# bcgsc/abyss

Measured on NVIDIA H100. Metric: k-mers/sec (Bloom insert + unitig extend), higher is better.
Workload: dtype u8

## Files before the change

abyss_b200/capi.py:

```python
from __future__ import annotations

import ctypes as C
import os

import numpy as np

_HERE = os.path.dirname(os.path.abspath(__file__))
LIB_PATH = os.path.join(_HERE, "lib", "libabyssb200.so")

ABB_OK, ABB_EINVAL, ABB_ENODEV, ABB_ECUDA, ABB_ENOMEM, ABB_ESTATE = 0, -1, -2, -3, -4, -5
COUNTING, BIT, CASCADING, KONNECTOR = 0, 1, 2, 3


class AbbError(RuntimeError):
    def __init__(self, code: int, msg: str):
        super().__init__(f"libabyssb200 error {code}: {msg}")
        self.code = code


class InsertStats(C.Structure):
    _fields_ = [("kmers", C.c_uint64), ("slots", C.c_uint64), ("windows", C.c_uint64),
                ("deferred", C.c_uint64), ("launches", C.c_uint64),
                ("ms_hash", C.c_float), ("ms_insert", C.c_float), ("ms_commit", C.c_float),
                ("commit_launches", C.c_uint64), ("commit_slots", C.c_uint64), ("drains", C.c_uint64),
                ("drained_slots", C.c_uint64), ("graph_launches", C.c_uint64), ("ms_graph", C.c_float)]


class Contig(C.Structure):
    _fields_ = [("seed_read", C.c_uint64), ("seq_offset", C.c_uint64),
                ("length", C.c_uint32), ("coverage", C.c_uint32)]


class AssemblyParams(C.Structure):
    _fields_ = [("trim", C.c_uint), ("verbose", C.c_uint), ("read_log", C.c_uint), ("reserved", C.c_uint)]


class TraceRow(C.Structure):
    _fields_ = [("contig_id", C.c_uint64), ("seed_read", C.c_uint64), ("length", C.c_uint32), ("seed_pos", C.c_uint32),
                ("left_n", C.c_uint32), ("right_n", C.c_uint32), ("left_code", C.c_uint8), ("right_code", C.c_uint8),
                ("redundant", C.c_uint8), ("pad", C.c_uint8)]


class AssemblyStats(C.Structure):
    _fields_ = [("rounds", C.c_uint64), ("speculated_reads", C.c_uint64), ("wasted_reads", C.c_uint64),
                ("candidates", C.c_uint64), ("contigs_tried", C.c_uint64), ("launches", C.c_uint64),
                ("ms_classify", C.c_float), ("ms_visited", C.c_float), ("ms_extend", C.c_float), ("ms_replay", C.c_float),
                ("ms_tiles", C.c_float), ("ms_walk", C.c_float), ("ms_stage", C.c_float), ("ms_repeat", C.c_float), ("ms_total", C.c_float), ("ms_cand", C.c_float), ("markers", C.c_uint64), ("tiles", C.c_uint64), ("serial_fallbacks", C.c_uint64),
                ("untiled_markers", C.c_uint64), ("dropped_tiles", C.c_uint64)]


class AssemblyCounters(C.Structure):
    _fields_ = [("solid_reads", C.c_uint64), ("visited_reads", C.c_uint64),
                ("reads_processed", C.c_uint64), ("bases_assembled", C.c_uint64),
                ("contig_id", C.c_uint64)]


class SuccInfo(C.Structure):
    _fields_ = [("hash", C.c_uint64 * 4), ("mask", C.c_uint8), ("pad", C.c_uint8 * 7)]


class NbrInfo(C.Structure):
    _fields_ = [("self", C.c_uint64), ("hash", C.c_uint64 * 8), ("attr", C.c_uint32), ("mask", C.c_uint8), ("pad", C.c_uint8 * 3)]


class OverlapEdge(C.Structure):
    _fields_ = [("u", C.c_uint32), ("v", C.c_uint32), ("distance", C.c_int32)]


class OverlapStats(C.Structure):
    _fields_ = [("vertices", C.c_uint64), ("exact_edges", C.c_uint64), ("short_edges", C.c_uint64), ("blunt_vertices", C.c_uint64),
                ("launches", C.c_uint64)]


_u64p = C.POINTER(C.c_uint64)
_u8p = C.POINTER(C.c_uint8)
_vp = C.c_void_p

SIGNATURES = {
    "abb_version": (C.c_int, []),
    "abb_last_error": (C.c_char_p, []),
    "abb_device_count": (C.c_int, []),
    "abb_filter_create": (C.c_int, [C.POINTER(_vp), C.c_int, C.c_uint64, C.c_uint, C.c_uint, C.c_uint, C.c_char_p, C.c_int]),
    "abb_filter_destroy": (C.c_int, [_vp]),
    "abb_konnector_create": (C.c_int, [C.POINTER(_vp), C.c_uint64, C.c_uint, C.c_uint, C.c_uint64, C.c_uint64, C.c_uint64, C.c_int]),
    "abb_filter_read_bits": (C.c_int, [_vp, C.c_int, _vp, C.c_uint64, C.c_uint64, C.c_int]),
    "abb_filter_compare": (C.c_int, [_vp, _vp, _u64p]),
    "abb_filter_level_popcount": (C.c_int, [_vp, C.c_int, _u64p]),
    "abb_filter_kmer_size": (C.c_uint, [_vp]),
    "abb_filter_hash_num": (C.c_uint, [_vp]),
    "abb_filter_size": (C.c_uint64, [_vp]),
    "abb_filter_size_in_bytes": (C.c_uint64, [_vp]),
    "abb_filter_threshold": (C.c_uint, [_vp]),
    "abb_filter_levels": (C.c_uint, [_vp]),
    "abb_filter_set_threshold": (C.c_int, [_vp, C.c_uint]),
    "abb_insert_reads": (C.c_int, [_vp, _vp, _vp, C.c_uint64, _u64p]),
    "abb_insert_reads_dev": (C.c_int, [_vp, _vp, _vp, C.c_uint64, C.c_uint64, _u64p]),
    "abb_insert_hashes": (C.c_int, [_vp, _vp, C.c_uint64]),
    "abb_contains_hashes": (C.c_int, [_vp, _vp, C.c_uint64, _vp]),
    "abb_mincount_hashes": (C.c_int, [_vp, _vp, C.c_uint64, _vp]),
    "abb_hash_reads": (C.c_int, [C.c_uint, C.c_char_p, _vp, _vp, C.c_uint64, _vp, _vp, _u64p, C.c_int]),
    "abb_hash_reads_dev": (C.c_int, [_vp, _vp, _vp, C.c_uint64, _vp, _vp, C.c_uint64, _u64p]),
    "abb_comm_unique_id": (C.c_int, [_vp]),
    "abb_comm_create": (C.c_int, [C.POINTER(_vp), C.c_int, C.c_int, _vp, C.c_int]),
    "abb_comm_destroy": (C.c_int, [_vp]),
    "abb_comm_rank": (C.c_int, [_vp]),
    "abb_comm_world": (C.c_int, [_vp]),
    "abb_insert_reads_sharded_dev": (C.c_int, [_vp, _vp, _vp, _vp, C.c_uint64, C.c_int, _u64p]),
    "abb_insert_reads_sharded": (C.c_int, [_vp, _vp, _vp, _vp, C.c_uint64, C.c_int, _u64p]),
    "abb_filter_resident_reads": (C.c_int, [_vp, C.POINTER(_vp), C.POINTER(_vp), _u64p]),
    "abb_filter_allgather": (C.c_int, [_vp, _vp]),
    "abb_comm_allgather_bytes": (C.c_int, [_vp, _vp, C.c_uint64, _vp]),
    "abb_comm_exchange_bytes": (C.c_int, [_vp, _vp, C.c_uint64, _vp, _u64p, _u64p, _vp]),
    "abb_filter_device_ptr": (_vp, [_vp, C.c_int]),
    "abb_filter_download": (C.c_int, [_vp, C.c_int, _vp, C.c_uint64]),
    "abb_filter_upload": (C.c_int, [_vp, C.c_int, _vp, C.c_uint64]),
    "abb_filter_clear": (C.c_int, [_vp]),
    "abb_filter_popcount": (C.c_int, [_vp, _u64p, _u64p]),
    "abb_assembler_create": (C.c_int, [C.POINTER(_vp), _vp, C.POINTER(AssemblyParams)]),
    "abb_assembler_destroy": (C.c_int, [_vp]),
    "abb_assembler_process_reads": (C.c_int, [_vp, _vp, _vp, C.c_uint64, C.POINTER(C.POINTER(Contig)), _u64p, C.POINTER(C.c_char_p)]),
    "abb_assembler_process_reads_dev": (C.c_int, [_vp, _vp, _vp, C.c_uint64, C.POINTER(C.POINTER(Contig)), _u64p, C.POINTER(C.c_char_p)]),
    "abb_assembler_stats": (C.c_int, [_vp, C.POINTER(AssemblyStats)]),
    "abb_assembler_reset": (C.c_int, [_vp]),
    "abb_assembler_counters": (C.c_int, [_vp, C.POINTER(AssemblyCounters)]),
    "abb_assembler_set_counters": (C.c_int, [_vp, C.POINTER(AssemblyCounters)]),
    "abb_assembler_read_results": (C.c_int, [_vp, C.POINTER(_u8p), _u64p]),
    "abb_assembler_set_comm": (C.c_int, [_vp, _vp]),
    "abb_assembler_trace": (C.c_int, [_vp, C.POINTER(C.POINTER(TraceRow)), _u64p]),
    "abb_assembler_assembled_filter": (_vp, [_vp]),
    "abb_filter_insert_stats": (C.c_int, [_vp, C.POINTER(InsertStats), C.c_int]),
# ... 441 lines not shown
```

abyss_b200/csrc/abb_assemble.cu:

```cuda
#include "abb_common.h"
#include "abb_walk.cuh"
#include <cooperative_groups.h>
#include <cub/device/device_select.cuh>
#include <thrust/iterator/counting_iterator.h>
#include <algorithm>
#include <chrono>
#include <cstdlib>
#include <cstring>
#include <new>
#include <vector>

namespace abb {
namespace cg = cooperative_groups;

__host__ __device__ inline uint64_t tile_slot(uint64_t key, unsigned cls, unsigned mask)
{
	return (((key ^ (0x9E3779B97F4A7C15ULL * (cls + 1))) * 0xD6E8FEB86659FD93ULL) >> 24) & mask;
}

struct WarpCtx {
	unsigned k, trim;
	RollTab rt;
	const HashCfg* cfg;
	const uint8_t* counters;
// ... 317 lines not shown
	unsigned ordinal;
	unsigned len;
	unsigned seed_pos;
	unsigned psize;
	unsigned char left, right, flags, pad1;
	unsigned long long front_h, back_h;
	unsigned left_n, right_n;
};

struct DevEmit {
	ContigRec* recs;
	unsigned* nrecs;
	unsigned cap;
	unsigned spec, ordinal;
	__device__ void operator()(WarpCtx& c, unsigned seed_pos, const ContigOut& o)
	{
		if (c.lane == 0) {
			const unsigned idx = atomicAdd(nrecs, 1u);
			if (idx < cap) {
				ContigRec r;
				r.seq = (unsigned long long)o.seq;
				r.spec = spec;
				r.ordinal = ordinal;
				r.len = o.len;
				r.seed_pos = seed_pos;
				r.psize = o.psize;
				r.left = (unsigned char)o.left;
				r.right = (unsigned char)o.right;
				r.flags = (unsigned char)((o.pushed_front ? 1 : 0) | (o.pushed_back ? 2 : 0) | (o.popped_front ? 4 : 0) | (o.popped_back ? 8 : 0));
				r.pad1 = 0;
				r.front_h = o.front_h;
				r.back_h = o.back_h;
				r.left_n = o.left_n;
				r.right_n = o.right_n;
				recs[idx] = r;
			}
		}
		++ordinal;
	}
};

struct IsCandidate {
	const uint8_t* codes;
	__host__ __device__ bool operator()(unsigned r) const { return codes[r] == RC_CANDIDATE; }
};

struct WalkCfg {
	unsigned k, trim, threshold;
	RollTab rt;
	const uint8_t* counters;
};

struct TileView {
	const TileRec* recs;
	const unsigned* tab;
	unsigned mask;
};

__device__ __forceinline__ WarpCtx make_ctx(const WalkCfg& w, const HashCfg* cfg, Frame* frames, uint64_t* look, unsigned gwarp,
                                            uint8_t* arena, unsigned long long arena_size, unsigned long long* arena_top)
{
	WarpCtx c;
	c.k = w.k;
	c.trim = w.trim;
	c.rt = w.rt;
	c.cfg = cfg;
	c.counters = w.counters;
	c.threshold = w.threshold;
	c.lane = threadIdx.x & 31;
	c.frames = frames ? frames + (size_t)gwarp * kFrameCap : nullptr;
	c.look = look + (size_t)gwarp * kLookCap;
	c.arena = arena;
	c.arena_size = arena_size;
	c.arena_top = arena_top;
	c.fail_ = 0;
	c.tile_recs = nullptr;
	c.tile_tab = nullptr;
	c.tile_mask = 0;
	return c;
}

constexpr int kWalkWarps = 4;

template <int KW>
__global__ void __launch_bounds__(kWalkWarps * 32)
k_classify(const uint8_t* __restrict__ bases, const uint64_t* __restrict__ offs, const uint64_t* __restrict__ slot_offs,
           const uint64_t* __restrict__ h0, const uint8_t* __restrict__ valid, uint64_t n_reads, WalkCfg w,
           const __grid_constant__ HashCfg cfg, uint64_t* look, int exact_codes, uint8_t* __restrict__ codes)
{
	const unsigned gwarp = blockIdx.x * kWalkWarps + (threadIdx.x >> 5);
	const unsigned nwarps = gridDim.x * kWalkWarps;
	WarpCtx c = make_ctx(w, &cfg, nullptr, look, gwarp, nullptr, 0, nullptr);
	const unsigned lane = c.lane;
	for (uint64_t r = gwarp; r < n_reads; r += nwarps) {
		const uint64_t beg = offs[r];
		const unsigned L = (unsigned)(offs[r + 1] - beg);
		uint8_t code;
		if (L < w.k) {
			code = RC_SHORTER_THAN_K;
		} else {
			const uint64_t s0 = slot_offs[r];
			const unsigned nk = L - w.k + 1;
			bool bad = false;
			if (w.rt.nmask) {
				for (unsigned j = lane; j < L; j += 32)
					bad |= base_code(bases[beg + j]) >= 4;
			} else
				for (unsigned j = lane; j < nk; j += 32)
					bad |= valid[s0 + j] == 0;
			if (__any_sync(0xffffffffu, bad)) {
				code = RC_NON_ACGT;
			} else {
				bool solid = true;
				for (unsigned base = 0; base < nk && solid; base += 32) {
					const unsigned j = base + lane;
					bool ok = true;
					if (j < nk) {
						const uint64_t h = h0[s0 + j];
						for (unsigned i = 0; i < cfg.H; ++i)
							ok &= __ldcg(w.counters + nth_pos(h, cfg, i)) >= w.threshold;
					}
					solid = __all_sync(0xffffffffu, ok);
				}
				if (!solid && !exact_codes) {
					code = RC_NOT_SOLID;
				} else {
					const Vtx<KW> first = vtx_from_codes<KW>(bases + beg, w.k, true, w.rt);
					bool blunt = !look_ahead(c, first, REV, kFpTrim);
					if (!blunt) {
						const Vtx<KW> last = vtx_from_codes<KW>(bases + beg + L - w.k, w.k, true, w.rt);
						blunt = !look_ahead(c, vtx_revcomp(last, w.k), REV, kFpTrim);
					}
					code = blunt ? RC_BLUNT_END : (solid ? RC_CANDIDATE : RC_NOT_SOLID);
				}
			}
		}
		if (lane == 0)
			codes[r] = code;
	}
}

__global__ void __launch_bounds__(256)
k_visited(const unsigned* __restrict__ cand, unsigned c0, unsigned n, const uint64_t* __restrict__ slot_offs,
          const uint64_t* __restrict__ h0, const __grid_constant__ HashCfg cfg, const uint8_t* __restrict__ bits,
          uint8_t* __restrict__ out)
{
	const unsigned gwarp = (blockIdx.x * blockDim.x + threadIdx.x) >> 5, lane = threadIdx.x & 31;
	if (gwarp >= n)
		return;
	const unsigned r = cand[c0 + gwarp];
	const uint64_t s0 = slot_offs[r];
	const unsigned nk = (unsigned)(slot_offs[r + 1] - s0);
	bool all = true;
	for (unsigned base = 0; base < nk && all; base += 32) {
		const unsigned j = base + lane;
		bool ok = true;
		if (j < nk) {
			const uint64_t h = h0[s0 + j];
			for (unsigned i = 0; i < cfg.H; ++i) {
				const uint64_t p = nth_pos(h, cfg, i);
				ok &= (__ldcg(bits + (p >> 3)) >> (p & 7)) & 1;
			}
		}
		all = __all_sync(0xffffffffu, ok);
	}
	if (lane == 0)
		out[gwarp] = all;
}

template <int KW>
__global__ void __launch_bounds__(kWalkWarps * 32)
k_extend(const uint8_t* __restrict__ bases, const uint64_t* __restrict__ offs, const unsigned* __restrict__ spec, unsigned n_spec,
         WalkCfg w, const __grid_constant__ HashCfg cfg, Frame* frames, uint64_t* look, uint8_t* arena,
         unsigned long long arena_size, unsigned long long* arena_top, ContigRec* recs, unsigned* nrecs, unsigned rec_cap,
         unsigned* __restrict__ status, TileView tv)
{
	const unsigned gwarp = blockIdx.x * kWalkWarps + (threadIdx.x >> 5);
	if (gwarp >= n_spec)
		return;
	WarpCtx c = make_ctx(w, &cfg, frames, look, gwarp, arena, arena_size, arena_top);
	c.tile_recs = tv.recs;
	c.tile_tab = tv.tab;
	c.tile_mask = tv.mask;
	const unsigned r = spec[gwarp];
	const uint64_t beg = offs[r];
	const unsigned L = (unsigned)(offs[r + 1] - beg);
	DevEmit emit = { recs, nrecs, rec_cap, gwarp, 0 };
	const bool ok = walk_read<KW>(c, bases + beg, L, emit);
	if (c.lane == 0)
		status[gwarp] = ok ? 0u : (c.fail_ ? c.fail_ : walk_fail_bit(WALK_FAIL_NO_CODE));
}


__global__ void __launch_bounds__(256)
k_find_markers(const uint64_t* __restrict__ h0, const uint8_t* __restrict__ valid, const uint64_t* __restrict__ slot_offs,
               uint64_t n_reads, uint64_t n_slots, WalkCfg w, const __grid_constant__ HashCfg cfg, unsigned long long* mset,
               unsigned mset_mask, unsigned long long* __restrict__ out , unsigned* n_out,
               unsigned out_cap, unsigned* n_no_room, unsigned world, unsigned rank)
{
	for (uint64_t s = (uint64_t)blockIdx.x * blockDim.x + threadIdx.x; s < n_slots; s += (uint64_t)gridDim.x * blockDim.x) {
		const uint64_t h = h0[s];
		if (!is_marker(h) || !valid[s])
			continue;
		if (world > 1 && (unsigned)((h >> 8) % world) != rank)
			continue;
		bool solid = true;
		for (unsigned i = 0; i < cfg.H; ++i)
			solid &= __ldcg(w.counters + nth_pos(h, cfg, i)) >= w.threshold;
		if (!solid)
			continue;
		const unsigned ins = marker_set_insert(mset, mset_mask, h);
		if (ins == MARKER_NO_ROOM)
			atomicAdd(n_no_room, 1u);
		if (ins != MARKER_FRESH)
			continue;
		uint64_t lo = 0, hi = n_reads;
		while (lo < hi) {
			const uint64_t mid = (lo + hi) / 2;
			if (slot_offs[mid + 1] <= s)
				lo = mid + 1;
			else
// ... 458 lines not shown
	unsigned seg_s = 0, seg_c = 0;
	for (unsigned b = 0; b <= n_big; ++b) {
		const unsigned c_big = b < n_big ? big[b] : n_contigs;
		if (blockIdx.x == 0)
			replay_segment(io, seg_s, seg_c, c_big, cfg, k, counters, bits, ends);
		__threadfence();
		grid.sync();
		if (b == n_big)
			break;
		const unsigned s_of = big_s[b];
		if (__ldcg(io.rcode + s_of) == RC_GENERATED_CONTIGS) {
			big_check(io, c_big, cfg, bits);
			__threadfence();
			grid.sync();
			if (__ldcg(io.caccept + c_big) != 0) {
				big_apply(io, c_big, cfg, counters, bits);
				__threadfence();
				grid.sync();
			}
		}
		seg_s = s_of;
		seg_c = c_big + 1;
	}
}

}

using namespace abb;

struct abb_assembler {
	abb_filter* solid = nullptr;
	std::unique_ptr<abb_filter, decltype(&abb_filter_destroy)> assembled{ nullptr, abb_filter_destroy };
	abb_assembly_params params = {};
	abb_assembly_counters counters = {};
	cudaStream_t stream = nullptr;
	uint64_t reads_seen = 0;
	int kw = 0;
	RollTab rt;
	DevBuf<uint8_t> d_mpos;
	abb_comm* comm = nullptr;
	DevBuf<uint8_t> gather;
	const uint8_t* cur_bases = nullptr;
	const uint64_t* cur_offs = nullptr;

	DevBuf<uint8_t> bases, valid, codes, vis, scan_tmp, cseq, cvalid, rcode, caccept;
	DevBuf<uint64_t> offs, slot_offs, h0, coffs, cslot, ch0;
	DevBuf<unsigned> cand, spec, spec_cbeg, clen, ccov, status, seg_contig, seg_len, big_idx, big_spec;
	DevBuf<uint64_t> seg_beg, seg_slot, rep_off;
	DevBuf<ContigRec> recs, recs_sorted;
	DevBuf<Frame> frames;
	DevBuf<uint64_t> look;
	unsigned scratch_warps = 0;
	DevBuf<uint8_t> d_arena;
	unsigned long long arena_size = 0;
	DevBuf<unsigned long long> d_arena_top;
	DevBuf<unsigned> d_nrecs;
	DevBuf<unsigned long long> d_ends;
	unsigned ends_cap = 0;
	DevBuf<unsigned> d_ends_n;
	uint64_t ends_upper = 0;

	bool tiles_on = true;
	DevBuf<TileRec> d_tiles;
	unsigned tile_cap = 0;
	DevBuf<unsigned> d_tile_tab;
	unsigned tile_tab_mask = 0;
	DevBuf<unsigned> d_tile_n;
	DevBuf<uint8_t> d_tile_pool;
	unsigned long long tile_pool_size = 0;
	DevBuf<unsigned long long> d_tile_pool_top;
	DevBuf<unsigned long long> d_marker_set;
	unsigned marker_set_mask = 0;
	DevBuf<unsigned long long> new_markers, rep_tab;
	DevBuf<TileRec> tile_export;
	DevBuf<uint8_t> stage_bases, rep_flag;
	DevBuf<uint64_t> stage_hashes;

	unsigned spec_target = 512;
	std::vector<abb_contig> out_contigs;
	std::vector<char> out_seqs;
	std::vector<uint8_t> out_codes;
	std::vector<abb_trace_row> out_trace;
	abb_assembly_stats st = {};
	unsigned sms = 0, tile_ctas = 0, replay_grid = 0;
	Event ev[2], ev2[2];

	unsigned world() const { return comm ? (unsigned)abb_comm_world(comm) : 1u; }
	unsigned rank() const { return comm ? (unsigned)abb_comm_rank(comm) : 0u; }
	StreamTimer time_phase(float* acc) { return StreamTimer(ev[0], ev[1], stream, acc); }
	StreamTimer time_inner(float* acc) { return StreamTimer(ev2[0], ev2[1], stream, acc); }
};

namespace {

constexpr unsigned kMaxSpec = 1024;
constexpr unsigned kTileCounters = 5;
constexpr unsigned kMinSpec = 256;
constexpr unsigned long long kArenaDefault = 4ULL << 30;
static unsigned long long g_arena_hint = 0;
constexpr unsigned long long kArenaMax = 96ULL << 30;

int ensure_scratch(abb_assembler* a, unsigned warps)
{
	if (warps <= a->scratch_warps)
		return ABB_OK;
	ABB_CHECK(a->frames.reserve((size_t)warps * kFrameCap));
	ABB_CHECK(a->look.reserve((size_t)warps * kLookCap));
	a->scratch_warps = warps;
	return ABB_OK;
}

int ensure_arena(abb_assembler* a, unsigned long long bytes)
{
	if (a->d_arena.p && a->arena_size >= bytes)
		return ABB_OK;
	a->arena_size = 0;
	ABB_CHECK(a->d_arena.alloc(bytes));
	a->arena_size = bytes;
	return ABB_OK;
}

int ensure_endset(abb_assembler* a, uint64_t extra)
{
	const uint64_t need = (a->ends_upper + extra) * 2 + 16;
	if (a->d_ends.p && need <= a->ends_cap)
		return ABB_OK;
	uint64_t ncap = a->ends_cap ? a->ends_cap : 1024;
	while (ncap < need)
		ncap <<= 1;
	ABB_REQUIRE(ncap <= (1ULL << 31), "contigEndKmers table too large");
	DevBuf<unsigned long long> nt;
	ABB_CHECK(nt.alloc(ncap));
	ABB_CUDA(cudaMemsetAsync(nt.p, 0, ncap * sizeof(unsigned long long), a->stream));
	if (a->d_ends.p) {
		k_endset_rehash<<<256, 256, 0, a->stream>>>(a->d_ends.p, a->ends_cap, nt.p, (unsigned)ncap);
		ABB_CUDA(cudaGetLastError());
		ABB_CUDA(cudaStreamSynchronize(a->stream));
	}
	a->d_ends = std::move(nt);
	a->ends_cap = (unsigned)ncap;
	return ABB_OK;
}

WalkCfg walk_cfg(const abb_assembler* a)
{
	WalkCfg w;
	w.k = a->solid->k;
	w.trim = a->params.trim;
	w.threshold = a->solid->threshold;
	w.rt = a->rt;
	w.counters = a->solid->d_data.p;
	return w;
}

#define ABB_DISPATCH_KW(kw, ...)              \
	do {                                      \
		switch (kw) {                         \
		case 1: { constexpr int KW = 1; __VA_ARGS__; } break; \
		case 2: { constexpr int KW = 2; __VA_ARGS__; } break; \
		case 3: { constexpr int KW = 3; __VA_ARGS__; } break; \
		case 4: { constexpr int KW = 4; __VA_ARGS__; } break; \
		default: { constexpr int KW = 6; __VA_ARGS__; } break; \
		}                                     \
	} while (0)

template <typename T>
int h2d(DevBuf<T>& d, const std::vector<T>& h, cudaStream_t s)
// ... 606 lines not shown
	if (r.n_ok == r.n_spec) {
		if (wasted * 2 <= r.n_ok)
			a->spec_target = std::min(kMaxSpec, a->spec_target * 2);
		else if (wasted * 20 > r.n_ok * 19)
			a->spec_target = std::max(kMinSpec, a->spec_target / 2);
	}
}

int speculate_round(abb_assembler* a, const std::vector<unsigned>& cand, size_t* cursor)
{
	Round r;
	ABB_CHECK(scan_uncovered(a, cand, cursor, r));
	if (r.spec.empty())
		return ABB_OK;
	++a->st.rounds;
	a->st.speculated_reads += r.n_spec;
	{
		StreamTimer te = a->time_phase(&a->st.ms_extend);
		ABB_CHECK(extend_tiled(a, r));
		ABB_CHECK(check_repeats(a, r));
		ABB_CHECK(serial_fallback(a, r));
		layout_records(r.recs, r.n_ok, a->solid->k, r.L);
		ABB_CHECK(stage_contigs(a, r.recs, r.L));
	}
	hand_back_failed(a, cand, cursor, r);
	ABB_CHECK(replay(a, r));
	collect(a, r);
	return ABB_OK;
}

}

extern "C" {

int abb_assembler_create(abb_assembler** out, abb_filter* solid, const abb_assembly_params* params)
{
	ABB_REQUIRE(out && solid && params, "NULL argument");
	*out = nullptr;
	if (solid->kind != ABB_COUNTING) {
		set_error("the assembler needs a counting filter (CountingBloomFilter<uint8_t>), like abyss-bloom-dbg");
		return ABB_ESTATE;
	}
	if (!solid->mask.empty()) {
		const std::string& m = solid->mask;
		ABB_REQUIRE(m.size() == solid->k, "spaced seed must be k characters long");
		ABB_REQUIRE(m.front() == '1' && m.back() == '1', "spaced seed must begin and end with '1's");
		ABB_REQUIRE(std::equal(m.begin(), m.end(), m.rbegin()), "spaced seed must be symmetric");
	}
	ABB_REQUIRE(solid->k >= 2, "k must be at least 2 for graph traversal");
	ABB_CUDA(cudaSetDevice(solid->device));
	std::unique_ptr<abb_assembler> a(new (std::nothrow) abb_assembler());
	if (!a) {
		set_error("out of host memory");
		return ABB_ENOMEM;
	}
	a->solid = solid;
	a->params = *params;
	if (a->params.trim == 0xffffffffu)
		a->params.trim = solid->k;
	a->kw = (int)((2 * solid->k + 63) / 64);
	a->rt = make_rolltab(solid->k);
	if (!solid->mask.empty()) {
		std::vector<uint8_t> mpos;
		for (unsigned i = 0; i < solid->k; ++i)
			if (solid->mask[i] == '0')
				mpos.push_back((uint8_t)i);
		if (!mpos.empty()) {
			if (a->d_mpos.alloc(mpos.size()) != ABB_OK ||
			    cudaMemcpy(a->d_mpos.p, mpos.data(), mpos.size(), cudaMemcpyHostToDevice) != cudaSuccess) {
				set_error("cudaMalloc of the spaced-seed table failed");
				return ABB_ECUDA;
			}
			a->rt.nmask = (unsigned)mpos.size();
			a->rt.mpos = a->d_mpos.p;
		}
	}
	a->tiles_on = getenv("ABB_NO_TILES") == nullptr && solid->mask.empty();
	abb_filter* assembled = nullptr;
	ABB_CHECK(abb_filter_create(&assembled, ABB_BIT, solid->size, solid->H, solid->k, 0, "", solid->device));
	a->assembled.reset(assembled);
	a->stream = solid->stream;
	a->sms = sm_count();
	int per_sm = 0;
	ABB_DISPATCH_KW(a->kw, ABB_CUDA(cudaOccupancyMaxActiveBlocksPerMultiprocessor(&per_sm, k_make_tiles<KW>, kWalkWarps * 32, 0)));
	a->tile_ctas = a->sms * (unsigned)std::max(1, per_sm);
	ABB_CUDA(cudaOccupancyMaxActiveBlocksPerMultiprocessor(&per_sm, k_replay_all, 1024, 0));
	a->replay_grid = a->sms * (unsigned)std::max(1, per_sm);
	for (Event* e : { &a->ev[0], &a->ev[1], &a->ev2[0], &a->ev2[1] })
		ABB_CUDA(cudaEventCreate(e->out()));
	ABB_CHECK(a->d_arena_top.alloc(1));
	ABB_CHECK(a->d_nrecs.alloc(1));
	ABB_CHECK(a->d_ends_n.alloc(2));
	ABB_CUDA(cudaMemset(a->d_ends_n.p, 0, 2 * sizeof(unsigned)));
	return hand_over(a, out);
}

int abb_assembler_destroy(abb_assembler* a)
{
	if (!a)
		return ABB_OK;
	cudaSetDevice(a->solid->device);
	cudaStreamSynchronize(a->stream);
	delete a;
	return ABB_OK;
}

static int hash_and_classify(abb_assembler* a, const uint8_t* d_bases, const uint64_t* d_offs, uint64_t n_reads, uint64_t* total_out)
{
	abb_filter* f = a->solid;
	cudaStream_t st = a->stream;
	uint64_t total = 0;
	ABB_CHECK(compute_slot_offsets(f->k, d_offs, n_reads, a->slot_offs, a->scan_tmp, st, &total, &a->st.launches));
	ABB_CHECK(a->h0.reserve(total + 1));
	ABB_CHECK(a->valid.reserve(total + 1));
	ABB_CHECK(a->codes.reserve(n_reads));
	if (total)
		ABB_CHECK(launch_hash(f->k, f->d_care.p, d_bases, d_offs, a->slot_offs.p, 0, n_reads, 0, a->h0.p, a->valid.p, st,
		                      &a->st.launches));
	*total_out = total;
	const auto [lo, up] = slice_of(n_reads, a->rank(), a->world());
	const unsigned grid = std::min(blocks_for(std::max<uint64_t>(up - lo, 1), kWalkWarps), a->sms * 8);
	ABB_CHECK(ensure_scratch(a, grid * kWalkWarps));
	const WalkCfg w = walk_cfg(a);
	if (up > lo)
		ABB_DISPATCH_KW(a->kw, (k_classify<KW><<<grid, kWalkWarps * 32, 0, st>>>(d_bases, d_offs + lo, a->slot_offs.p + lo, a->h0.p, a->valid.p,
		                                                                        up - lo, w, f->cfg, a->look.p, (int)a->params.read_log,
		                                                                        a->codes.p + lo)));
	ABB_CUDA(cudaGetLastError());
	++a->st.launches;
	if (a->world() > 1)
		ABB_CHECK(allgather_slices(a, a->codes.p + lo, n_reads, a->codes.p));
	return ABB_OK;
}

static int process_batch(abb_assembler* a, const uint8_t* d_bases, const uint64_t* d_offs, uint64_t n_reads,
                         const abb_contig** contigs, uint64_t* n_contigs, const char** seqs)
{
	const auto t_begin = std::chrono::steady_clock::now();
	struct Total {
		abb_assembler* a;
		std::chrono::steady_clock::time_point t0;
		~Total() { a->st.ms_total += std::chrono::duration<float, std::milli>(std::chrono::steady_clock::now() - t0).count(); }
	} total_guard{ a, t_begin };
	cudaStream_t st = a->stream;
	a->cur_bases = d_bases;
	a->cur_offs = d_offs;
	uint64_t total = 0;
	{
		StreamTimer tc = a->time_phase(&a->st.ms_classify);
		ABB_CHECK(hash_and_classify(a, d_bases, d_offs, n_reads, &total));
		ABB_CUDA(cudaMemcpyAsync(a->out_codes.data(), a->codes.p, n_reads, cudaMemcpyDeviceToHost, st));
		ABB_CUDA(cudaStreamSynchronize(st));
	}

	const auto t_cand = std::chrono::steady_clock::now();
	std::vector<unsigned> cand;
	{
		ABB_CHECK(a->cand.reserve(n_reads + 1));
		IsCandidate pred{ a->codes.p };
		thrust::counting_iterator<unsigned> first(0);
		size_t bytes = 0;
		ABB_CUDA(cub::DeviceSelect::If(nullptr, bytes, first, a->cand.p, a->d_nrecs.p, (int)n_reads, pred, st));
		ABB_CHECK(a->scan_tmp.reserve(bytes));
		ABB_CUDA(cub::DeviceSelect::If(a->scan_tmp.p, bytes, first, a->cand.p, a->d_nrecs.p, (int)n_reads, pred, st));
		unsigned nc = 0;
		ABB_CUDA(cudaMemcpyAsync(&nc, a->d_nrecs.p, sizeof nc, cudaMemcpyDeviceToHost, st));
		ABB_CUDA(cudaStreamSynchronize(st));
		cand.resize(nc);
		if (nc)
			ABB_CUDA(cudaMemcpyAsync(cand.data(), a->cand.p, (size_t)nc * sizeof(unsigned), cudaMemcpyDeviceToHost, st));
		ABB_CUDA(cudaStreamSynchronize(st));
	}
	a->st.ms_cand += std::chrono::duration<float, std::milli>(std::chrono::steady_clock::now() - t_cand).count();
	a->counters.solid_reads += cand.size();
	a->st.candidates += cand.size();
	if (!cand.empty())
		ABB_CHECK(produce_tiles(a, n_reads, total));

	size_t cursor = 0;
	while (cursor < cand.size())
		ABB_CHECK(speculate_round(a, cand, &cursor));

	a->counters.reads_processed += n_reads;
	a->reads_seen += n_reads;
	if (contigs) *contigs = a->out_contigs.data();
	if (n_contigs) *n_contigs = a->out_contigs.size();
	if (seqs) *seqs = a->out_seqs.data();
	return ABB_OK;
}

static int begin_batch(abb_assembler* a, uint64_t n_reads, const abb_contig** contigs, uint64_t* n_contigs, const char** seqs)
{
	ABB_REQUIRE(a, "NULL assembler");
	a->out_contigs.clear();
	a->out_seqs.clear();
	a->out_trace.clear();
	a->out_codes.assign(n_reads, RC_SHORTER_THAN_K);
	if (contigs) *contigs = nullptr;
	if (n_contigs) *n_contigs = 0;
	if (seqs) *seqs = nullptr;
	ABB_REQUIRE(n_reads < (1ULL << 31), "at most 2^31-1 reads per batch");
	ABB_CUDA(cudaSetDevice(a->solid->device));
	ABB_CUDA(cudaStreamSynchronize(a->solid->stream));
	ABB_CUDA(cudaStreamSynchronize(a->assembled->stream));
	return ABB_OK;
}

int abb_assembler_process_reads(abb_assembler* a, const char* bases, const uint64_t* offsets, uint64_t n_reads,
                                const abb_contig** contigs, uint64_t* n_contigs, const char** seqs)
{
	ABB_CHECK(begin_batch(a, n_reads, contigs, n_contigs, seqs));
// ... 94 lines not shown
```

include/abyss_b200.h:

```cpp
#ifndef ABYSS_B200_H
#define ABYSS_B200_H

#include <stddef.h>
#include <stdint.h>

#ifdef __cplusplus
extern "C" {
#endif

#define ABB_VERSION 101

enum {
	ABB_OK = 0,
	ABB_EINVAL = -1,
	ABB_ENODEV = -2,
	ABB_ECUDA = -3,
	ABB_ENOMEM = -4,
	ABB_ESTATE = -5
};

enum {
	ABB_COUNTING = 0,
	ABB_BIT = 1,
	ABB_CASCADING = 2,
// ... 40 lines not shown
                   uint64_t n_reads, uint64_t* out_h0, uint8_t* out_valid, uint64_t* n_slots_out,
                   int device);

int abb_hash_reads_dev(abb_filter* f, const char* d_bases, const uint64_t* d_offsets, uint64_t n_reads,
                       uint64_t* d_h0, uint8_t* d_valid, uint64_t capacity, uint64_t* n_slots_out);

typedef struct abb_comm abb_comm;
int abb_comm_unique_id(uint8_t id_out[128]);
int abb_comm_create(abb_comm** out, int rank, int world, const uint8_t id[128], int device);
int abb_comm_destroy(abb_comm* c);
int abb_comm_rank(const abb_comm* c);
int abb_comm_world(const abb_comm* c);
int abb_insert_reads_sharded_dev(abb_filter* f, abb_comm* c, const char* d_bases, const uint64_t* d_offsets, uint64_t n_reads,
                                 int finalize, uint64_t* n_kmers_out);
int abb_insert_reads_sharded(abb_filter* f, abb_comm* c, const char* bases, const uint64_t* offsets, uint64_t n_reads, int finalize,
                             uint64_t* n_kmers_out);
int abb_filter_allgather(abb_filter* f, abb_comm* c);
int abb_filter_resident_reads(abb_filter* f, const char** d_bases, const uint64_t** d_offsets, uint64_t* n_reads);
int abb_comm_allgather_bytes(abb_comm* c, void* d_buf, uint64_t bytes_per_rank, void* cuda_stream);
int abb_comm_exchange_bytes(abb_comm* c, const void* d_send, uint64_t send_bytes, void* d_recv_base, const uint64_t* recv_offsets,
                            const uint64_t* recv_bytes, void* cuda_stream);

void* abb_filter_device_ptr(abb_filter* f, int level);

int abb_filter_download(abb_filter* f, int level, uint8_t* host, uint64_t nbytes);
int abb_filter_upload(abb_filter* f, int level, const uint8_t* host, uint64_t nbytes);
int abb_filter_clear(abb_filter* f);

int abb_filter_popcount(abb_filter* f, uint64_t* nonzero, uint64_t* at_or_above_threshold);

typedef struct abb_assembly_params {
	unsigned trim;
	unsigned verbose;
	unsigned read_log;
	unsigned reserved;
} abb_assembly_params;

typedef struct abb_contig {
	uint64_t seed_read;
	uint64_t seq_offset;
	uint32_t length;
	uint32_t coverage;
} abb_contig;

typedef struct abb_assembly_counters {
	uint64_t solid_reads, visited_reads, reads_processed, bases_assembled, contig_id;
} abb_assembly_counters;

int abb_assembler_create(abb_assembler** out, abb_filter* solid, const abb_assembly_params* params);
int abb_assembler_destroy(abb_assembler* a);
int abb_assembler_process_reads(abb_assembler* a, const char* bases, const uint64_t* offsets,
                                uint64_t n_reads, const abb_contig** contigs, uint64_t* n_contigs,
                                const char** seqs);
int abb_assembler_process_reads_dev(abb_assembler* a, const char* d_bases, const uint64_t* d_offsets,
                                    uint64_t n_reads, const abb_contig** contigs, uint64_t* n_contigs,
                                    const char** seqs);
int abb_assembler_reset(abb_assembler* a);
int abb_assembler_counters(const abb_assembler* a, abb_assembly_counters* out);
int abb_assembler_set_counters(abb_assembler* a, const abb_assembly_counters* in);
int abb_assembler_read_results(const abb_assembler* a, const uint8_t** codes, uint64_t* n);
int abb_assembler_set_comm(abb_assembler* a, abb_comm* comm);
typedef struct abb_trace_row {
	uint64_t contig_id;
	uint64_t seed_read;
	uint32_t length;
	uint32_t seed_pos;
	uint32_t left_n, right_n;
	uint8_t left_code, right_code, redundant, pad;
} abb_trace_row;
int abb_assembler_trace(const abb_assembler* a, const abb_trace_row** rows, uint64_t* n);
abb_filter* abb_assembler_assembled_filter(abb_assembler* a);

typedef struct abb_assembly_stats {
	uint64_t rounds;
	uint64_t speculated_reads;
	uint64_t wasted_reads;
	uint64_t candidates;
	uint64_t contigs_tried;
	uint64_t launches;
	float ms_classify, ms_visited, ms_extend, ms_replay;
	float ms_tiles;
	float ms_walk, ms_stage, ms_repeat;
	float ms_total, ms_cand;
	uint64_t markers, tiles;
	uint64_t serial_fallbacks;
	uint64_t untiled_markers;
	uint64_t dropped_tiles;
} abb_assembly_stats;
int abb_assembler_stats(const abb_assembler* a, abb_assembly_stats* out);

int abb_contains_reads(abb_filter* f, const char* bases, const uint64_t* offsets, uint64_t n_reads, uint8_t* out_flag,
                       uint8_t* out_valid, uint64_t capacity, uint64_t* n_slots_out);

typedef struct abb_succ_info {
	uint64_t hash[4];
	uint8_t mask;
	uint8_t pad[7];
} abb_succ_info;
int abb_successors(abb_filter* f, const char* kmers, uint64_t n, unsigned max_chain, abb_succ_info* out, unsigned* out_len,
                   uint64_t* self_hash);

typedef struct abb_nbr_info {
	uint64_t self;
	uint64_t hash[8];
	uint32_t attr;
	uint8_t mask;
	uint8_t pad[3];
} abb_nbr_info;
int abb_graph_neighbors(abb_filter* graph, const char* kmers, uint64_t n, abb_filter* const* attr, unsigned n_attr, abb_nbr_info* out);

typedef struct abb_overlap abb_overlap;
typedef struct abb_overlap_edge {
	uint32_t u, v;
	int32_t distance;
} abb_overlap_edge;
typedef struct abb_overlap_stats {
	uint64_t vertices, exact_edges, short_edges, blunt_vertices, launches;
} abb_overlap_stats;
int abb_overlap_create(abb_overlap** out, int device);
int abb_overlap_destroy(abb_overlap* h);
int abb_overlap_build(abb_overlap* h, const char* bases, const uint64_t* offsets, uint64_t n_contigs, unsigned k,
                      unsigned min_overlap, int ss, const abb_overlap_edge** edges, uint64_t* n_edges);
int abb_overlap_get_stats(const abb_overlap* h, abb_overlap_stats* out);

typedef struct abb_insert_stats {
	uint64_t kmers;
	uint64_t slots;
	uint64_t windows;
	uint64_t deferred;
	uint64_t launches;
	float ms_hash, ms_insert;
	float ms_commit;
	uint64_t commit_launches;
	uint64_t commit_slots;
	uint64_t drains;
	uint64_t drained_slots;
	uint64_t graph_launches;
	float ms_graph;
} abb_insert_stats;
int abb_filter_insert_stats(abb_filter* f, abb_insert_stats* out, int reset);
int abb_filter_set_profiling(abb_filter* f, int on);
void* abb_filter_stream(abb_filter* f);
int abb_filter_set_window(abb_filter* f, uint64_t window_slots);

#ifdef __cplusplus
}
#endif
#endif
```

Before: 715.3 million.

## Split read classification into solidity kernel, compaction, and half-warp blunt-end test

The monolithic classify kernel becomes a lightweight solidity kernel that batches several k-mers and hashes per lane, so more Bloom counter loads are in flight at once. Only reads that still need a blunt-end check are then compacted with cub DeviceSelect and handed to a separate kernel. That kernel checks both read ends at the same time, using a half-warp per end with a new HalfCtx. The aim is to avoid warp divergence and wasted look-ahead work on non-solid reads, and to raise memory-level parallelism. In exchange it adds extra launches, a selection pass, a larger look scratch buffer and an ABI change to the stats struct.

```diff
diff --git a/abyss_b200/capi.py b/abyss_b200/capi.py
--- a/abyss_b200/capi.py
+++ b/abyss_b200/capi.py
@@ -45,7 +45,8 @@
     _fields_ = [("rounds", C.c_uint64), ("speculated_reads", C.c_uint64), ("wasted_reads", C.c_uint64),
                 ("candidates", C.c_uint64), ("contigs_tried", C.c_uint64), ("launches", C.c_uint64),
                 ("ms_classify", C.c_float), ("ms_visited", C.c_float), ("ms_extend", C.c_float), ("ms_replay", C.c_float),
-                ("ms_tiles", C.c_float), ("ms_walk", C.c_float), ("ms_stage", C.c_float), ("ms_repeat", C.c_float), ("ms_total", C.c_float), ("ms_cand", C.c_float), ("markers", C.c_uint64), ("tiles", C.c_uint64), ("serial_fallbacks", C.c_uint64),
+                ("ms_tiles", C.c_float), ("ms_walk", C.c_float), ("ms_stage", C.c_float), ("ms_repeat", C.c_float), ("ms_total", C.c_float), ("ms_cand", C.c_float),
+                ("ms_solid", C.c_float), ("ms_blunt", C.c_float), ("markers", C.c_uint64), ("tiles", C.c_uint64), ("serial_fallbacks", C.c_uint64),
                 ("untiled_markers", C.c_uint64), ("dropped_tiles", C.c_uint64)]
 
 
diff --git a/abyss_b200/csrc/abb_assemble.cu b/abyss_b200/csrc/abb_assemble.cu
--- a/abyss_b200/csrc/abb_assemble.cu
+++ b/abyss_b200/csrc/abb_assemble.cu
@@ -423,27 +423,29 @@
 
 constexpr int kWalkWarps = 4;
 
-template <int KW>
-__global__ void __launch_bounds__(kWalkWarps * 32)
-k_classify(const uint8_t* __restrict__ bases, const uint64_t* __restrict__ offs, const uint64_t* __restrict__ slot_offs,
-           const uint64_t* __restrict__ h0, const uint8_t* __restrict__ valid, uint64_t n_reads, WalkCfg w,
-           const __grid_constant__ HashCfg cfg, uint64_t* look, int exact_codes, uint8_t* __restrict__ codes)
-{
-	const unsigned gwarp = blockIdx.x * kWalkWarps + (threadIdx.x >> 5);
-	const unsigned nwarps = gridDim.x * kWalkWarps;
-	WarpCtx c = make_ctx(w, &cfg, nullptr, look, gwarp, nullptr, 0, nullptr);
-	const unsigned lane = c.lane;
-	for (uint64_t r = gwarp; r < n_reads; r += nwarps) {
+constexpr unsigned kSolidThreads = 256;
+constexpr unsigned kSolidKmersPerLane = 4;
+constexpr unsigned kSolidHashes = 4;
+constexpr unsigned kSolidFirst = 32;
+
+__global__ void __launch_bounds__(kSolidThreads)
+k_solid(const uint8_t* __restrict__ bases, const uint64_t* __restrict__ offs, const uint64_t* __restrict__ slot_offs,
+        const uint64_t* __restrict__ h0, const uint8_t* __restrict__ valid, uint64_t n_reads, unsigned k, unsigned nmask,
+        const uint8_t* __restrict__ counters, unsigned threshold, const __grid_constant__ HashCfg cfg, uint8_t* __restrict__ codes)
+{
+	const unsigned lane = threadIdx.x & 31;
+	const uint64_t nwarps = (uint64_t)gridDim.x * (kSolidThreads / 32);
+	for (uint64_t r = ((uint64_t)blockIdx.x * kSolidThreads + threadIdx.x) >> 5; r < n_reads; r += nwarps) {
 		const uint64_t beg = offs[r];
 		const unsigned L = (unsigned)(offs[r + 1] - beg);
 		uint8_t code;
-		if (L < w.k) {
+		if (L < k) {
 			code = RC_SHORTER_THAN_K;
 		} else {
 			const uint64_t s0 = slot_offs[r];
-			const unsigned nk = L - w.k + 1;
+			const unsigned nk = L - k + 1;
 			bool bad = false;
-			if (w.rt.nmask) {
+			if (nmask) {
 				for (unsigned j = lane; j < L; j += 32)
 					bad |= base_code(bases[beg + j]) >= 4;
 			} else
@@ -453,31 +455,102 @@
 				code = RC_NON_ACGT;
 			} else {
 				bool solid = true;
-				for (unsigned base = 0; base < nk && solid; base += 32) {
-					const unsigned j = base + lane;
+				for (unsigned base = 0, span = kSolidFirst; base < nk && solid; base += span, span = 32 * kSolidKmersPerLane) {
+					const unsigned end = min(nk, base + span);
+					uint64_t h[kSolidKmersPerLane];
+#pragma unroll
+					for (unsigned t = 0; t < kSolidKmersPerLane; ++t) {
+						const unsigned j = base + lane + 32 * t;
+						h[t] = j < end ? h0[s0 + j] : 0;
+					}
 					bool ok = true;
-					if (j < nk) {
-						const uint64_t h = h0[s0 + j];
-						for (unsigned i = 0; i < cfg.H; ++i)
-							ok &= __ldcg(w.counters + nth_pos(h, cfg, i)) >= w.threshold;
+					for (unsigned i0 = 0; i0 < cfg.H; i0 += kSolidHashes) {
+						unsigned v[kSolidKmersPerLane][kSolidHashes];
+#pragma unroll
+						for (unsigned t = 0; t < kSolidKmersPerLane; ++t)
+#pragma unroll
+							for (unsigned d = 0; d < kSolidHashes; ++d)
+								v[t][d] = base + lane + 32 * t < end && i0 + d < cfg.H ? __ldcg(counters + nth_pos(h[t], cfg, i0 + d)) : 255u;
+#pragma unroll
+						for (unsigned t = 0; t < kSolidKmersPerLane; ++t)
+#pragma unroll
+							for (unsigned d = 0; d < kSolidHashes; ++d)
+								ok &= v[t][d] >= threshold;
 					}
 					solid = __all_sync(0xffffffffu, ok);
 				}
-				if (!solid && !exact_codes) {
-					code = RC_NOT_SOLID;
-				} else {
-					const Vtx<KW> first = vtx_from_codes<KW>(bases + beg, w.k, true, w.rt);
-					bool blunt = !look_ahead(c, first, REV, kFpTrim);
-					if (!blunt) {
-						const Vtx<KW> last = vtx_from_codes<KW>(bases + beg + L - w.k, w.k, true, w.rt);
-						blunt = !look_ahead(c, vtx_revcomp(last, w.k), REV, kFpTrim);
-					}
-					code = blunt ? RC_BLUNT_END : (solid ? RC_CANDIDATE : RC_NOT_SOLID);
-				}
+				code = solid ? RC_CANDIDATE : RC_NOT_SOLID;
 			}
 		}
 		if (lane == 0)
 			codes[r] = code;
+	}
+}
+
+struct NeedsBluntTest {
+	const uint8_t* codes;
+	bool exact;
+	__host__ __device__ bool operator()(unsigned r) const { return codes[r] == RC_CANDIDATE || (exact && codes[r] == RC_NOT_SOLID); }
+};
+
+struct HalfCtx {
+	unsigned k;
+	RollTab rt;
+	const HashCfg* cfg;
+	const uint8_t* counters;
+	unsigned threshold;
+	unsigned lane;
+	unsigned shift;
+	uint64_t* look;
+
+	__device__ unsigned mask() const { return 0xffffu << shift; }
+	template <int KW>
+	__device__ unsigned neighbors_dir(const Vtx<KW>& v, Dir d) const
+	{
+		const unsigned n = lane >> 2, hs = lane & 3;
+		const uint64_t h0 = neighbor_bloom(v, k, rt, d, n);
+		unsigned mn = 255;
+		for (unsigned i = hs; i < cfg->H; i += 4)
+			mn = min(mn, (unsigned)__ldcg(counters + nth_pos(h0, *cfg, i)));
+		unsigned b = __ballot_sync(mask(), mn >= threshold) >> shift;
+		b &= b >> 1;
+		b &= b >> 2;
+		return (b & 1u) | ((b >> 3) & 2u) | ((b >> 6) & 4u) | ((b >> 9) & 8u);
+	}
+	__device__ void wr64(uint64_t* p, uint64_t v) const { *(volatile uint64_t*)p = v; }
+	__device__ void sync() const { __syncwarp(mask()); }
+	__device__ bool find64(const uint64_t* a, unsigned n, uint64_t key, unsigned stride) const
+	{
+		for (unsigned base = 0; base < n; base += 16) {
+			const unsigned i = base + lane;
+			const bool hit = i < n && *(const volatile uint64_t*)(a + (size_t)i * stride) == key;
+			if (__any_sync(mask(), hit))
+				return true;
+		}
+		return false;
+	}
+	__device__ void fail(unsigned) {}
+};
+
+template <int KW>
+__global__ void __launch_bounds__(kWalkWarps * 32)
+k_blunt(const uint8_t* __restrict__ bases, const uint64_t* __restrict__ offs, const unsigned* __restrict__ sel,
+        const unsigned* __restrict__ n_sel, WalkCfg w, const __grid_constant__ HashCfg cfg, uint64_t* look, uint8_t* __restrict__ codes)
+{
+	const unsigned gwarp = blockIdx.x * kWalkWarps + (threadIdx.x >> 5), nwarps = gridDim.x * kWalkWarps;
+	const unsigned lane = threadIdx.x & 31, half = lane >> 4;
+	HalfCtx c = { w.k, w.rt, &cfg, w.counters, w.threshold, lane & 15, 16 * half, look + ((size_t)gwarp * 2 + half) * kLookCap };
+	const unsigned n = *n_sel;
+	for (unsigned i = gwarp; i < n; i += nwarps) {
+		const unsigned r = sel[i];
+		const uint64_t beg = offs[r];
+		const unsigned L = (unsigned)(offs[r + 1] - beg);
+		Vtx<KW> v = vtx_from_codes<KW>(bases + beg + (half ? L - w.k : 0), w.k, true, w.rt);
+		if (half)
+			v = vtx_revcomp(v, w.k);
+		const bool ok = look_ahead(c, v, REV, kFpTrim);
+		if (__ballot_sync(0xffffffffu, !ok) != 0 && lane == 0)
+			codes[r] = RC_BLUNT_END;
 	}
 }
 
@@ -1102,7 +1175,7 @@
 	std::vector<uint8_t> out_codes;
 	std::vector<abb_trace_row> out_trace;
 	abb_assembly_stats st = {};
-	unsigned sms = 0, tile_ctas = 0, replay_grid = 0;
+	unsigned sms = 0, solid_ctas = 0, blunt_ctas = 0, tile_ctas = 0, replay_grid = 0;
 	Event ev[2], ev2[2];
 
 	unsigned world() const { return comm ? (unsigned)abb_comm_world(comm) : 1u; }
@@ -1875,6 +1948,10 @@
 	a->stream = solid->stream;
 	a->sms = sm_count();
 	int per_sm = 0;
+	ABB_CUDA(cudaOccupancyMaxActiveBlocksPerMultiprocessor(&per_sm, k_solid, kSolidThreads, 0));
+	a->solid_ctas = a->sms * (unsigned)std::max(1, per_sm);
+	ABB_DISPATCH_KW(a->kw, ABB_CUDA(cudaOccupancyMaxActiveBlocksPerMultiprocessor(&per_sm, k_blunt<KW>, kWalkWarps * 32, 0)));
+	a->blunt_ctas = a->sms * (unsigned)std::max(1, per_sm);
 	ABB_DISPATCH_KW(a->kw, ABB_CUDA(cudaOccupancyMaxActiveBlocksPerMultiprocessor(&per_sm, k_make_tiles<KW>, kWalkWarps * 32, 0)));
 	a->tile_ctas = a->sms * (unsigned)std::max(1, per_sm);
 	ABB_CUDA(cudaOccupancyMaxActiveBlocksPerMultiprocessor(&per_sm, k_replay_all, 1024, 0));
@@ -1912,14 +1989,31 @@
 		                      &a->st.launches));
 	*total_out = total;
 	const auto [lo, up] = slice_of(n_reads, a->rank(), a->world());
-	const unsigned grid = std::min(blocks_for(std::max<uint64_t>(up - lo, 1), kWalkWarps), a->sms * 8);
-	ABB_CHECK(ensure_scratch(a, grid * kWalkWarps));
-	const WalkCfg w = walk_cfg(a);
-	if (up > lo)
-		ABB_DISPATCH_KW(a->kw, (k_classify<KW><<<grid, kWalkWarps * 32, 0, st>>>(d_bases, d_offs + lo, a->slot_offs.p + lo, a->h0.p, a->valid.p,
-		                                                                        up - lo, w, f->cfg, a->look.p, (int)a->params.read_log,
-		                                                                        a->codes.p + lo)));
-	ABB_CUDA(cudaGetLastError());
+	const uint64_t n = up - lo;
+	if (n) {
+		StreamTimer ts = a->time_inner(&a->st.ms_solid);
+		k_solid<<<std::min(blocks_for(n * 32, kSolidThreads), a->solid_ctas), kSolidThreads, 0, st>>>(
+		    d_bases, d_offs + lo, a->slot_offs.p + lo, a->h0.p, a->valid.p, n, f->k, a->rt.nmask, f->d_data.p, f->threshold, f->cfg,
+		    a->codes.p + lo);
+		ABB_CUDA(cudaGetLastError());
+	}
+	if (n) {
+		StreamTimer tb = a->time_inner(&a->st.ms_blunt);
+		ABB_CHECK(a->cand.reserve(n + 1));
+		NeedsBluntTest pred{ a->codes.p + lo, a->params.read_log != 0 };
+		thrust::counting_iterator<unsigned> first(0);
+		size_t bytes = 0;
+		ABB_CUDA(cub::DeviceSelect::If(nullptr, bytes, first, a->cand.p, a->d_nrecs.p, (int)n, pred, st));
+		ABB_CHECK(a->scan_tmp.reserve(bytes));
+		ABB_CUDA(cub::DeviceSelect::If(a->scan_tmp.p, bytes, first, a->cand.p, a->d_nrecs.p, (int)n, pred, st));
+		const unsigned grid = std::min(blocks_for(n, kWalkWarps), a->blunt_ctas);
+		ABB_CHECK(a->look.reserve((size_t)grid * kWalkWarps * 2 * kLookCap));
+		const WalkCfg w = walk_cfg(a);
+		ABB_DISPATCH_KW(a->kw, (k_blunt<KW><<<grid, kWalkWarps * 32, 0, st>>>(d_bases, d_offs + lo, a->cand.p, a->d_nrecs.p, w, f->cfg,
+		                                                                    a->look.p, a->codes.p + lo)));
+		ABB_CUDA(cudaGetLastError());
+		a->st.launches += 2;
+	}
 	++a->st.launches;
 	if (a->world() > 1)
 		ABB_CHECK(allgather_slices(a, a->codes.p + lo, n_reads, a->codes.p));
diff --git a/include/abyss_b200.h b/include/abyss_b200.h
--- a/include/abyss_b200.h
+++ b/include/abyss_b200.h
@@ -146,6 +146,7 @@
 	float ms_tiles;
 	float ms_walk, ms_stage, ms_repeat;
 	float ms_total, ms_cand;
+	float ms_solid, ms_blunt;
 	uint64_t markers, tiles;
 	uint64_t serial_fallbacks;
 	uint64_t untiled_markers;
```

Measured after the change: 730.7 million (median of 6 runs). 2.1% higher.
